# jens-nau/NeRF-VO

Hardware: AMD Instinct MI355X
Metric: training ray-samples/sec (higher is better)
Workload: dtype f16; 1 GPU; BASELINE configs[1]: Replica-shaped full mapping step, depth-nerfacto (proposal sampling 256/96/48), fixed poses; normal_supervision=False, loss_scale=GradScaler 65536 dynamic, skipped_zero_weight_heads=True, rays_per_gpu=4096, samples_per_ray=48, keyframes=192, sampler=proposal-network (nerfacto), parallelism=single GPU (no process group)

## Files before the change

include/nerfvo_hip.h:

```cpp
#ifndef NERFVO_HIP_H
#define NERFVO_HIP_H

#include <stddef.h>
#include <stdint.h>

#ifdef __cplusplus
extern "C" {
#endif

#define NVO_OK 0
#define NVO_ERR_INVALID 1
#define NVO_ERR_HIP 2
#define NVO_ERR_UNSUPPORTED 3

typedef struct nvo_module_s* nvo_module_t;
typedef void* nvo_stream_t;

const char* nvo_last_error(void);
int nvo_version(void);
int nvo_profile_enable(int on);
int64_t nvo_profile_summary(char* buf, uint64_t buf_size);

int nvo_create_encoding(uint32_t n_input_dims, const char* encoding_json, nvo_module_t* out);
int nvo_create_network(uint32_t n_input_dims, uint32_t n_output_dims, const char* network_json,
// ... 132 lines not shown
    uint32_t R, S, S_out;
    const void* pre;
    uint32_t pre_stride;
    const float* x01;
    const float* sbins;
    const float* tbins;
    float density_bias;
    float* sigma;
    float* weights;
    float anneal, histogram_padding, near_plane, far_plane;
    const float* jitter;
    float* sbins_out;
    float* tbins_out;
    const float* anneal_dev;
    const float* origins;
    const float* directions;
    float* x01_out;
    int act_bf16;
} nvo_weights_pdf_args;
int nvo_weights_pdf(nvo_stream_t stream, const nvo_weights_pdf_args* args);

typedef struct nvo_main_loss_args {
    uint32_t R, S;
    const void* pre;
    uint32_t pre_stride;
    const void* rgb;
    uint32_t rgb_stride;
    const float* x01;
    const float* sbins;
    const float* tbins;
    float density_bias;
    const float* gt_rgb;
    const float* gt_depth;
    const float* directions_norm;
    float rgb_mult, distortion_mult, depth_mult, depth_sigma;
    float inv_rays;
    float depth_level_div;
    float loss_scale;
    float* out_rgb;
    float* out_depth;
    float* out_expected_depth;
    float* out_accumulation;
    float* weights;
    float* losses;
    void* dpre;
    uint32_t dpre_stride;
    void* drgb;
    uint32_t drgb_stride;
    const float* dsigma_dx;
    float dsigma_inv_scale;
    const float* gt_normal;
    float normal_mult;
    float* out_normals;
    int act_bf16;
    const float* loss_scale_dev;
    uint32_t* nonfinite_flag;
    uint8_t* tile_live;
} nvo_main_loss_args;
int nvo_main_render_loss(nvo_stream_t stream, const nvo_main_loss_args* args);

typedef struct nvo_prop_loss_args {
    uint32_t R, S, S_main;
    const void* pre;
    uint32_t pre_stride;
    const float* x01;
    const float* sbins;
    const float* tbins;
    const float* sbins_main;
    const float* weights_main;
    float density_bias;
    const float* gt_depth;
    const float* directions_norm;
    float interlevel_mult, depth_mult, depth_sigma;
    float inv_rays, depth_level_div, loss_scale;
    float* losses;
    void* dpre;
    uint32_t dpre_stride;
    int act_bf16;
    const float* loss_scale_dev;
    uint32_t* nonfinite_flag;
} nvo_prop_loss_args;
int nvo_prop_loss(nvo_stream_t stream, const nvo_prop_loss_args* args);
int nvo_prop_loss_pair(nvo_stream_t stream, const nvo_prop_loss_args* args0, const nvo_prop_loss_args* args1);

typedef struct nvo_color_args {
    uint32_t R, S;
    const void* sh;
    const void* base_out;
    const void* embedding;
    const int32_t* cam_idx;
    const void* weights;
    void* rgb;
    void* hidden;
    const void* drgb;
    void* d_base_out;
    float* d_embedding;
    float* d_sh;
    float* d_weights;
    int act_bf16;
    void* det_scratch;
    uint64_t det_scratch_bytes;
    uint32_t n_cameras;
    uint32_t* nonfinite_flag;
    float* dw_replicas;
    uint32_t n_dw_replicas;
    const uint8_t* tile_live;
    const float* tile_live_count;
} nvo_color_args;
int nvo_nerfacto_color_fwd(nvo_stream_t stream, const nvo_color_args* args);
int nvo_nerfacto_color_bwd(nvo_stream_t stream, const nvo_color_args* args);
uint64_t nvo_color_det_scratch_bytes(uint32_t R, uint32_t S);

uint64_t nvo_occ_march_scratch_bytes(uint32_t R);
int nvo_occ_march(nvo_stream_t stream, uint32_t R, const float* origins, const float* directions,
                  const uint8_t* bitfield, int n_levels, float cone_angle, float t_near, const float* jitter,
                  uint32_t capacity, uint32_t* counts, uint32_t* offsets, int32_t* ray_idx, float* t_out,
                  float* dt_out, void* scratch, uint64_t scratch_bytes);
int nvo_occ_march_resume(nvo_stream_t stream, uint32_t R, const float* origins, const float* directions,
                         const uint8_t* bitfield, int n_levels, float cone_angle, float t_near, const float* jitter,
                         uint32_t capacity, uint32_t* counts, uint32_t* offsets, int32_t* ray_idx, float* t_out,
                         float* dt_out, void* scratch, uint64_t scratch_bytes, const float* t_resume, uint32_t max_new,
                         float* t_next);
int nvo_occ_march_runs(nvo_stream_t stream, uint32_t R, const float* origins, const float* directions,
                       const uint8_t* bitfield, int n_levels, float cone_angle, float t_near, const float* jitter,
                       uint32_t* counts, void* scratch, uint64_t scratch_bytes, const float* t_resume, uint32_t max_new,
                       float* t_next, const uint32_t* R_dev, uint32_t run_offset);
int nvo_occ_pack(nvo_stream_t stream, uint32_t R, const uint32_t* counts_in, uint32_t capacity, uint32_t* counts_out,
                 uint32_t* offsets, uint32_t* totals, const void* scratch, uint64_t scratch_bytes, int32_t* ray_idx,
                 float* t_out, float* dt_out, const uint32_t* R_dev, uint32_t run_offset);
uint64_t nvo_occ_pack_state_bytes(void);
int nvo_occ_pack_fused(nvo_stream_t stream, uint32_t R, const uint32_t* counts_in, uint32_t capacity, uint32_t* counts_out,
                       uint32_t* offsets, uint32_t* totals, const void* scratch, uint64_t scratch_bytes, int32_t* ray_idx,
                       float* t_out, float* dt_out, const uint32_t* R_dev, uint32_t run_offset, void* state,
                       const float* origins, const float* directions, float aabb_lo, float aabb_hi, float* x01,
                       uint32_t rays_per_group );
int nvo_occ_update(nvo_stream_t stream, int n_levels, float* grid, const float* fresh, float decay,
                   float threshold, uint8_t* bitfield, void* scratch8);
int nvo_occ_cell_positions(nvo_stream_t stream, int level, const float* jitter, float* positions);
int nvo_occ_mark_untrained(nvo_stream_t stream, int n_levels, float* grid, uint32_t n_images, const float* intrinsics,
                           const float* c2w, uint32_t H, uint32_t W, float margin);
int nvo_occ_sample_cells(nvo_stream_t stream, uint32_t n, uint32_t first, uint32_t n_total, uint32_t step, uint32_t seed,
                         uint32_t stream_id, int n_levels, const float* grid, float thresh, float aabb_lo, float aabb_hi,
                         float* x01, uint32_t* cell_idx);

typedef struct nvo_ngp_rgb_args {
    uint32_t capacity;
    const void* sh;
    const void* density_out;
    const int32_t* ray_idx;
    const void* weights;
    void* rgb_out;
    void* hidden;
    const void* d_rgb_out;
    void* d_density_out;
    const float* d_density_pre;
    float* d_weights;
    uint32_t* nonfinite_flag;
    float* dw_replicas;
    uint32_t n_dw_replicas;
} nvo_ngp_rgb_args;
int nvo_ngp_rgb_fwd(nvo_stream_t stream, const nvo_ngp_rgb_args* args);
int nvo_ngp_rgb_bwd(nvo_stream_t stream, const nvo_ngp_rgb_args* args);

typedef struct nvo_ngp_loss_args {
    uint32_t R, capacity;
    const uint32_t* counts;
// ... 209 lines not shown
```

nerf-vo_amd/_lib.py:

```python
from __future__ import annotations

import ctypes as C
import os
from pathlib import Path

PKG_DIR = Path(__file__).resolve().parent
LIB_PATH = PKG_DIR / "lib" / "libnerfvo_hip.so"

_lib = None

_u32, _u64, _i64, _int = C.c_uint32, C.c_uint64, C.c_int64, C.c_int
_i32 = C.c_int32
_p = C.c_void_p
_f = C.c_float


class WeightsPdfArgs(C.Structure):
    _fields_ = [("R", _u32), ("S", _u32), ("S_out", _u32), ("pre", _p), ("pre_stride", _u32), ("x01", _p),
                ("sbins", _p), ("tbins", _p), ("density_bias", _f), ("sigma", _p), ("weights", _p),
                ("anneal", _f), ("histogram_padding", _f), ("near_plane", _f), ("far_plane", _f),
                ("jitter", _p), ("sbins_out", _p), ("tbins_out", _p), ("anneal_dev", _p),
                ("origins", _p), ("directions", _p), ("x01_out", _p), ("act_bf16", _int)]


# ... 69 lines not shown
                ("nonfinite_flag", _p), ("dw_replicas", _p), ("n_dw_replicas", _u32)]


class NgpLossArgs(C.Structure):
    _fields_ = [("R", _u32), ("capacity", _u32), ("counts", _p), ("offsets", _p), ("ray_idx", _p), ("t", _p), ("dt", _p),
                ("density_out", _p), ("density_stride", _u32), ("rgb_out", _p), ("rgb_stride", _u32),
                ("background", _p), ("gt_rgb", _p), ("gt_depth", _p), ("directions_norm", _p), ("rgb_mult", _f),
                ("depth_mult", _f), ("inv_rays", _f), ("loss_scale", _f), ("out_rgb", _p), ("out_depth", _p),
                ("out_accumulation", _p), ("losses", _p), ("d_rgb_out", _p), ("d_rgb_stride", _u32),
                ("d_density_pre", _p), ("carry_in", _p), ("carry_out", _p), ("accumulate_outputs", _u32),
                ("train_min_transmittance", _f), ("gt_depth_cov", _p), ("ray_state", _p), ("R_dev", _p), ("world_size", _u32)]


class NgpAliveArgs(C.Structure):
    _fields_ = [("R", _u32), ("counts", _p), ("offsets", _p), ("dt", _p), ("density_out", _p), ("density_stride", _u32),
                ("min_transmittance", _f), ("kept", _p), ("state", _p), ("R_dev", _p), ("resume_in", _p), ("carry_in", _p),
                ("kept_base", _u32), ("t_next", _p), ("resume_out", _p), ("carry_out", _p)]


class TsdfArgs(C.Structure):
    _fields_ = [("tsdf", _p), ("weight", _p), ("color", _p), ("frames", _p), ("depth", _p), ("rgb", _p),
                ("nx", _u32), ("ny", _u32), ("nz", _u32), ("K", _u32), ("H", _u32), ("W", _u32),
                ("lower_x", _f), ("lower_y", _f), ("lower_z", _f), ("voxel_size", _f), ("trunc", _f), ("depth_max", _f)]


TSDF_MAX_FRAMES = 16


class NnArgs(C.Structure):
    _fields_ = [("points", _p), ("point_index", _p), ("cell_start", _p), ("queries", _p), ("out_dist2", _p), ("out_index", _p),
                ("N", _u32), ("M", _u32), ("gx", _u32), ("gy", _u32), ("gz", _u32),
                ("lower_x", _f), ("lower_y", _f), ("lower_z", _f), ("cell_size", _f), ("max_dist", _f),
                ("has_xf", _i32), ("xf", _f * 12)]


NN_MAX_CELLS_PER_AXIS = 1024


_SIGNATURES = {
    "nvo_last_error": (C.c_char_p, []),
    "nvo_version": (_int, []),
    "nvo_profile_enable": (_int, [_int]),
    "nvo_profile_summary": (_i64, [C.c_char_p, _u64]),
    "nvo_create_encoding": (_int, [_u32, C.c_char_p, C.POINTER(_p)]),
    "nvo_create_network": (_int, [_u32, _u32, C.c_char_p, C.POINTER(_p)]),
    "nvo_create_network_with_input_encoding": (_int, [_u32, _u32, C.c_char_p, C.c_char_p, C.POINTER(_p)]),
    "nvo_destroy": (_int, [_p]),
    "nvo_n_input_dims": (_u32, [_p]),
    "nvo_n_output_dims": (_u32, [_p]),
    "nvo_padded_output_dims": (_u32, [_p]),
    "nvo_n_params": (_u64, [_p]),
    "nvo_initial_params": (_int, [_p, _u64, _p]),
    "nvo_ctx_bytes": (_u64, [_p, _u32]),
    "nvo_set_option": (_int, [_p, C.c_char_p, _i64]),
    "nvo_fwd": (_int, [_p, _p, _u32, _p, _p, _p, _p]),
    "nvo_bwd": (_int, [_p, _p, _u32, _p, _p, _p, _p, _p, _p, _p]),
    "nvo_bwd_fork": (_int, [_p, _p, _p, _u32, _p, _p, _p, _p, _p, _p, _p]),
    "nvo_grid_describe": (_int, [_p, _p, _p]),
    "nvo_grid_indices": (_int, [_p, _p, _u32, _p, _p]),
    "nvo_raygen": (_int, [_p, _u32, _p, _p, _p, _p, _p, _p, _p, _p, _p]),
    "nvo_se3_exp_map": (_int, [_p, _u32, _p, _p]),
    "nvo_pose_exp_map": (_int, [_p, _u32, _p, _p, _int]),
    "nvo_positions_bwd": (_int, [_p, _u32, _u32, _p, _p, _p, _p, _p, _p]),
    "nvo_sh_bwd_input_f32": (_int, [_p, _u32, _u32, _p, _p, _p]),
    "nvo_pose_bwd": (_int, [_p, _u32, _p, _p, _p, _p, _p, _p, _p]),
    "nvo_se3_exp_map_bwd": (_int, [_p, _u32, _p, _p, _f, _f, _f, _p, _p, _int]),
    "nvo_se3_exp_map_bwd_scaled": (_int, [_p, _u32, _p, _p, _f, _f, _f, _p, _p, _int, _p]),
    "nvo_gather_pixels": (_int, [_p, _u32, _p, _u32, _u32, _u32, _p, _p]),
    "nvo_sample_lindisp": (_int, [_p, _u32, _u32, _f, _f, _p, _p, _p]),
    "nvo_sample_pixels": (_int, [_p, _u32, _u32, _p, _p, _p, _p, _u32]),
    "nvo_lindisp_positions": (_int, [_p, _u32, _u32, _f, _f, _p, _p, _p, _p, _p, _p]),
    "nvo_gather_targets": (_int, [_p, _u32, _p, _u32, _u32, _p, _p, _p, _p, _p, _p, _p, _p]),
    "nvo_sample_positions": (_int, [_p, _u32, _u32, _p, _p, _p, _p]),
    "nvo_dirs01": (_int, [_p, _u32, _p, _p]),
    "nvo_sh_encode": (_int, [_p, _u32, _u32, _p, _p]),
    "nvo_sh_encode_t": (_int, [_p, _u32, _u32, _p, _p, _int]),
    "nvo_ray_head": (_int, [_p, C.POINTER(RayHeadArgs)]),
    "nvo_rays_given": (_int, [_p, _u32, _p, _p, _p, _p, _u32, _u32, _p, _p, _p, _p, _p, _p, _p, _p, _p, _p, _p, _p, _p, _p]),
    "nvo_ray_head_zero": (_int, [_p, C.POINTER(RayHeadArgs), _u32, _p, _p]),
    "nvo_weights_pdf": (_int, [_p, C.POINTER(WeightsPdfArgs)]),
    "nvo_main_render_loss": (_int, [_p, C.POINTER(MainLossArgs)]),
    "nvo_prop_loss": (_int, [_p, C.POINTER(PropLossArgs)]),
    "nvo_prop_loss_pair": (_int, [_p, _p, _p]),
    "nvo_nerfacto_color_fwd": (_int, [_p, C.POINTER(ColorArgs)]),
    "nvo_nerfacto_color_bwd": (_int, [_p, C.POINTER(ColorArgs)]),
    "nvo_color_det_scratch_bytes": (_u64, [_u32, _u32]),
    "nvo_pose_bwd_cams": (_int, [_p, _u32, _p, _p, _p, _p, _p, _p, _p, _u32]),
    "nvo_pose_bwd_det": (_int, [_p, _u32, _p, _p, _p, _p, _p, _p, _p, _p, _u32]),
    "nvo_occ_march_scratch_bytes": (_u64, [_u32]),
    "nvo_occ_march": (_int, [_p, _u32, _p, _p, _p, _int, _f, _f, _p, _u32, _p, _p, _p, _p, _p, _p, _u64]),
    "nvo_occ_march_resume": (_int, [_p, _u32, _p, _p, _p, _int, _f, _f, _p, _u32, _p, _p, _p, _p, _p, _p, _u64, _p, _u32, _p]),
    "nvo_occ_update": (_int, [_p, _int, _p, _p, _f, _f, _p, _p]),
    "nvo_occ_cell_positions": (_int, [_p, _int, _p, _p]),
    "nvo_occ_mark_untrained": (_int, [_p, _int, _p, _u32, _p, _p, _u32, _u32, _f]),
    "nvo_occ_sample_cells": (_int, [_p, _u32, _u32, _u32, _u32, _u32, _u32, _int, _p, _f, _f, _f, _p, _p]),
    "nvo_occ_march_runs": (_int, [_p, _u32, _p, _p, _p, _int, _f, _f, _p, _p, _p, _u64, _p, _u32, _p, _p, _u32]),
    "nvo_occ_pack": (_int, [_p, _u32, _p, _u32, _p, _p, _p, _p, _u64, _p, _p, _p, _p, _u32]),
    "nvo_occ_pack_state_bytes": (_u64, []),
    "nvo_occ_pack_fused": (_int, [_p, _u32, _p, _u32, _p, _p, _p, _p, _u64, _p, _p, _p, _p, _u32, _p, _p, _p, _f, _f, _p, _u32]),
    "nvo_ngp_count_alive": (_int, [_p, C.POINTER(NgpAliveArgs)]),
    "nvo_ngp_positions_live": (_int, [_p, _u32, _p, _p, _p, _p, _f, _f, _p, _p]),
    "nvo_ngp_positions_bwd_dev": (_int, [_p, _u32, _u32, _p, _p, _p, _p, _p, _f, _f, _p, _p, _p, _p]),
    "nvo_ngp_positions": (_int, [_p, _u32, _p, _p, _p, _p, _f, _f, _p]),
    "nvo_depth_align_scratch_bytes": (_u64, [_u32, _u32]),
    "nvo_depth_align": (_int, [_p, C.POINTER(DepthAlignArgs)]),
    "nvo_ngp_positions_bwd": (_int, [_p, _u32, _u32, _p, _p, _p, _p, _p, _f, _f, _p, _p, _p]),
    "nvo_ngp_rgb_fwd": (_int, [_p, C.POINTER(NgpRgbArgs)]),
    "nvo_ngp_rgb_bwd": (_int, [_p, C.POINTER(NgpRgbArgs)]),
    "nvo_ngp_composite_loss": (_int, [_p, C.POINTER(NgpLossArgs)]),
    "nvo_ngp_thickness": (_int, [_p, _u32, _p, _u32, _int, _p]),
    "nvo_ngp_thickness_splat": (_int, [_p, _u32, _p, _u32, _p, _p]),
    "nvo_fill_i32": (_int, [_p, _u32, _p, _i32]),
    "nvo_tsdf_integrate": (_int, [_p, C.POINTER(TsdfArgs)]),
    "nvo_nn_query": (_int, [_p, C.POINTER(NnArgs)]),
    "nvo_adam_step": (_int, [_p, _u64, _p, _p, _p, _int, _p, _p, _f, _f, _f, _f, _u32, _f, _f, _p, _p]),
    "nvo_write_floats": (_int, [_p, _p, _u32, _p]),
    "nvo_nonfinite_flag": (_int, [_p, _u64, _p, _int, _p]),
    "nvo_nonfinite_flag_or": (_int, [_p, _u64, _p, _int, _p]),
    "nvo_adam_step_groups": (_int, [_p, _u32, _p, _p, _p, _p, _int, _p, _p, _f, _f, _f, _f, _f, _p]),
    "nvo_nonfinite_flag_ranges": (_int, [_p, _u32, _p, _p, _p, _int, _p]),
    "nvo_nonfinite_flag_ranges_or": (_int, [_p, _u32, _p, _p, _p, _int, _p]),
    "nvo_nonfinite_flag_spans_or": (_int, [_p, _u32, _p, _p, _p, _p, _int, _p]),
    "nvo_cast_half": (_int, [_p, _u64, _p, _p]),
    "nvo_zero_ranges": (_int, [_p, _u32, _p, _p]),
    "nvo_bwd_zero_ranges": (_int, [_p, _p, _p, _p, _u32]),
    "nvo_fold_replicas": (_int, [_p, _u32, _p, _p, _p, _p]),
    "nvo_fused_adam_range": (_int, [_p, _p, _p]),
    "nvo_set_fused_adam": (_int, [_p, _p]),
    "nvo_ema_update": (_int, [_p, _u64, _p, _p, _p, _f, _u32, _p]),
    "nvo_ema_update_dev": (_int, [_p, _u64, _p, _p, _p, _f, _p, _p]),
    "nvo_ema_update_dev_part": (_int, [_p, _u64, _p, _p, _p, _f, _p, _p]),
    "nvo_cast_working_copy": (_int, [_p, _u64, _p, _p, _u32, _p, _p]),
    "nvo_adam_step_groups_mixed": (_int, [_p, _u32, _p, _p, _p, _p, _int, _p, _p, _f, _f, _f, _f, _f, _p, _u32, _p, _p]),
    "nvo_adam_step_groups_scaled": (_int, [_p, _u32, _p, _p, _p, _p, _int, _p, _p, _f, _f, _f, _f, _f, _p, _u32, _p, _p, _p]),
    "nvo_adam_step_groups_tail": (_int, [_p, _u32, _p, _p, _p, _p, _int, _p, _p, _f, _f, _f, _f, _f, _p, _u32, _p, _p, _p, _p]),
    "nvo_opt_commit_write": (_int, [_p, _u32, _u32, _u32, _p, _p, _p, _p, _f, _f, _u32, _f, _f, _p, _f, _f, _p, _u32, _p]),
    "nvo_opt_commit_table": (_int, [_p, _u32, _u32, _u32, _p, _p, _p, _p, _f, _f, _u32, _f, _f, _p, _f, _f, _p, _p, _u32, _p]),
    "nvo_opt_commit": (_int, [_p, _u32, _u32, _u32, _p, _p, _p, _p, _f, _f, _u32, _f, _f, _p, _f, _f]),
    "nvo_cast_bf16": (_int, [_p, _u64, _p, _p]),
    "nvo_cast_shards": (_int, [_p, _u64, _u32, _u32, _p, _p, _int, _p]),
    "nvo_flag_from_wire": (_int, [_p, _p, _p]),
}


def exported_symbols() -> list[str]:
    return sorted(_SIGNATURES)


def lib() -> C.CDLL:
    global _lib
    if _lib is None:
        if not LIB_PATH.exists():
            raise RuntimeError(
                f"{LIB_PATH} is missing: the HIP extension has not been built. "
                "Run `python -c 'import __graft_entry__ as g; g.build()'` (or `python nerf-vo_amd/build.py`). "
                "There is no CPU fallback."
            )
        import torch

        handle = C.CDLL(str(LIB_PATH), mode=getattr(os, "RTLD_NOW", 2))
        for name, (restype, argtypes) in _SIGNATURES.items():
            fn = getattr(handle, name)
            fn.restype = restype
            fn.argtypes = argtypes
        _lib = handle
    return _lib
# ... 7 lines not shown
```

nerf-vo_amd/csrc/render.hip:

```cpp
#include "nvo_kernels.h"
#include "../../include/nerfvo_hip.h"

#include <float.h>

namespace {

constexpr int kRayBlock = 256;
constexpr int kRaysPerBlock = kRayBlock / 64;
constexpr int kMaxS = 256;
constexpr float kLossEps = 1.0e-7f;

__device__ __forceinline__ float wave_incl_scan(float v, int) { return nvo_wave_incl_scan(v); }
__device__ __forceinline__ float wave_sum(float v) { return nvo_wave_sum(v); }

__device__ __forceinline__ float nan_to_num(float v) {
    if (isnan(v)) return 0.f;
    if (isinf(v)) return v > 0.f ? FLT_MAX : -FLT_MAX;
    return v;
}

__device__ __forceinline__ float spacing_fn(float x) { return x < 1.f ? x * 0.5f : 1.f - 1.f / (2.f * x); }
__device__ __forceinline__ float spacing_fn_inv(float x) { return x < 0.5f ? 2.f * x : 1.f / (2.f - 2.f * x); }

__device__ __forceinline__ int upper_bound(const float* a, int n, float v) {
// ... 409 lines not shown
    const float* x01 = a.x01 + 3 * so;
    ray_weights(lane, S, pre, bf, a.pre_stride, x01, tb, a.density_bias, nullptr, w, Tr);
    __builtin_amdgcn_fence(__ATOMIC_RELEASE, "wavefront");
    __builtin_amdgcn_wave_barrier();
    __builtin_amdgcn_fence(__ATOMIC_ACQUIRE, "wavefront");

    float carry = 0.f;
    for (uint32_t base = 0; base < S; base += 64) {
        const uint32_t i = base + lane;
        const float v = (i < S) ? w[i] : 0.f;
        const float incl = wave_incl_scan(v, lane) + carry;
        if (i < S) cy[i + 1] = incl;
        carry = nvo_wave_bcast(incl, 63);
    }
    if (lane == 0) cy[0] = 0.f;
    for (uint32_t i = lane; i < S + 2; i += 64) g[i] = 0.f;
    __builtin_amdgcn_fence(__ATOMIC_RELEASE, "wavefront");
    __builtin_amdgcn_wave_barrier();
    __builtin_amdgcn_fence(__ATOMIC_ACQUIRE, "wavefront");

    float l_inter = 0.f;
    if ((uint32_t)lane < Sm) {
        const float* cm = a.sbins_main + (size_t)r * (Sm + 1);
        const float wm = a.weights_main[(size_t)r * Sm + lane];
        int lo = upper_bound(sb, (int)S, cm[lane]) - 1;
        lo = min(max(lo, 0), (int)S - 1);
        int hi = upper_bound(sb + 1, (int)S, cm[lane + 1]);
        hi = min(max(hi, 0), (int)S - 1);
        const float w_outer = cy[hi + 1] - cy[lo];
        const float diff = wm - w_outer;
        if (diff > 0.f) {
            l_inter = diff * diff / (wm + kLossEps);
            const float coef = a.interlevel_mult * a.inv_rays / (float)Sm;
            const float gi = -2.f * diff / (wm + kLossEps) * coef;
            atomicAdd(&g[lo], gi);
            atomicAdd(&g[hi + 1], -gi);
        }
    }
    l_inter = wave_sum(l_inter) * a.inv_rays / (float)Sm;
    __builtin_amdgcn_fence(__ATOMIC_RELEASE, "wavefront");
    __builtin_amdgcn_wave_barrier();
    __builtin_amdgcn_fence(__ATOMIC_ACQUIRE, "wavefront");
    float l_depth = 0.f;
    const bool use_depth = a.depth_mult != 0.f && a.gt_depth;
    const float z = use_depth ? a.gt_depth[r] * a.directions_norm[r] : 0.f;
    const float mask = z > 0.f ? 1.f : 0.f;
    carry = 0.f;
    for (uint32_t base = 0; base < S; base += 64) {
        const uint32_t i = base + lane;
        const float v = (i < S) ? g[i] : 0.f;
        const float incl = wave_incl_scan(v, lane) + carry;
        carry = nvo_wave_bcast(incl, 63);
        float gi = incl;
        if (i < S && use_depth) {
            const float midp = 0.5f * (tb[i] + tb[i + 1]);
            const float len = tb[i + 1] - tb[i];
            const float gss = __expf(-((midp - z) * (midp - z)) / (2.f * a.depth_sigma)) * len * mask;
            l_depth += -__logf(w[i] + kLossEps) * gss;
            gi += a.depth_mult * a.depth_level_div * a.inv_rays * (-gss / (w[i] + kLossEps));
        }
        if (i < S) g[i] = gi;
    }
    l_depth = wave_sum(l_depth) * a.inv_rays * a.depth_level_div;
    if (lane == 0) {
        float* shard = a.losses + 8 * (r & 63u);
        atomicAdd(shard + 0, a.interlevel_mult * l_inter);
        atomicAdd(shard + 1, a.depth_mult * l_depth);
    }
    if (a.dpre == nullptr) return;
    __builtin_amdgcn_fence(__ATOMIC_RELEASE, "wavefront");
    __builtin_amdgcn_wave_barrier();
    __builtin_amdgcn_fence(__ATOMIC_ACQUIRE, "wavefront");
    const bool overflow = ray_weights_bwd(lane, S, pre, bf, a.pre_stride, x01, tb, a.density_bias, w, Tr, g, a.loss_scale,
                                          (nvo_h16*)a.dpre + so * a.dpre_stride, a.dpre_stride, true);
    if (a.nonfinite_flag && __ballot(overflow) != 0ull && lane == 0) atomicOr(a.nonfinite_flag, 1u);
    if (a.dpre_stride != 16) {
        for (uint32_t i = lane; i < S; i += 64) {
            nvo_h16* dp = (nvo_h16*)a.dpre + (so + i) * a.dpre_stride;
            for (uint32_t k = 1; k < a.dpre_stride; ++k) dp[k] = (nvo_h16)0;
        }
    }
}

}

extern "C" {

int nvo_weights_pdf(nvo_stream_t stream, const nvo_weights_pdf_args* args) {
    NVO_REQUIRE(args != nullptr, "weights_pdf: args is NULL");
    const nvo_weights_pdf_args a = *args;
    NVO_REQUIRE(a.S >= 1 && a.S <= (uint32_t)kMaxS, "weights_pdf: samples per ray %u not in 1..%d", a.S, kMaxS);
    NVO_REQUIRE(a.S_out <= (uint32_t)kMaxS, "weights_pdf: S_out %u > %d", a.S_out, kMaxS);
    NVO_REQUIRE(a.S_out == 0 || (a.sbins_out && a.tbins_out), "weights_pdf: output bins are NULL");
    NVO_REQUIRE(a.pre && a.x01 && a.tbins && a.weights && a.sbins, "weights_pdf: NULL input");
    NVO_REQUIRE(!a.x01_out || (a.origins && a.directions && a.S_out > 0), "weights_pdf: x01_out needs origins, directions and S_out");
    if (a.R == 0) return NVO_OK;
    NVO_PROF(stream, "weights_pdf[S%u]", a.S);
    NVO_LAUNCH(k_weights_pdf, dim3(nvo_div_up(a.R, kRaysPerBlock)), dim3(kRayBlock), 0,
                       (hipStream_t)stream, a);
    NVO_CHECK_LAUNCH();
    return NVO_OK;
}

int nvo_main_render_loss(nvo_stream_t stream, const nvo_main_loss_args* args) {
    NVO_REQUIRE(args != nullptr, "main_render_loss: args is NULL");
    const nvo_main_loss_args a = *args;
    NVO_REQUIRE(a.S >= 1 && a.S <= 64, "main_render_loss: samples per ray %u not in 1..64", a.S);
    NVO_REQUIRE(a.pre && a.rgb && a.x01 && a.sbins && a.tbins && a.out_rgb && a.out_depth &&
                a.out_accumulation, "main_render_loss: NULL input/output");
    NVO_REQUIRE(!a.dpre || (a.drgb && a.losses && a.gt_rgb && a.drgb_stride >= 3),
                "main_render_loss: training mode needs drgb, losses, gt_rgb");
    NVO_REQUIRE(!a.tile_live || (a.dpre && (a.S & 15u) == 0u), "main_render_loss: tile_live needs training mode and S %% 16 == 0 (S = %u)", a.S);
    if (a.R == 0) return NVO_OK;
    NVO_PROF(stream, "main_render_loss");
    NVO_LAUNCH(k_main_render_loss, dim3(nvo_div_up(a.R, kRaysPerBlock)), dim3(kRayBlock), 0,
                       (hipStream_t)stream, a);
    NVO_CHECK_LAUNCH();
    return NVO_OK;
}

int nvo_prop_loss(nvo_stream_t stream, const nvo_prop_loss_args* args) {
    NVO_REQUIRE(args != nullptr, "prop_loss: args is NULL");
    const nvo_prop_loss_args a = *args;
    NVO_REQUIRE(a.S >= 1 && a.S <= (uint32_t)kMaxS && a.S_main >= 1 && a.S_main <= 64,
                "prop_loss: S=%u (<=%d) S_main=%u (<=64)", a.S, kMaxS, a.S_main);
    NVO_REQUIRE(a.pre && a.x01 && a.sbins && a.tbins && a.sbins_main && a.weights_main && a.losses &&
                (a.dpre == nullptr || a.dpre_stride >= 1), "prop_loss: NULL input/output");
    if (a.R == 0) return NVO_OK;
    NVO_PROF(stream, "prop_loss[S%u]", a.S);
    const uint32_t blocks = nvo_div_up(a.R, kRaysPerBlock);
    NVO_LAUNCH(k_prop_loss, dim3(blocks), dim3(kRayBlock), 0, (hipStream_t)stream, a, a, blocks);
    NVO_CHECK_LAUNCH();
    return NVO_OK;
}

int nvo_prop_loss_pair(nvo_stream_t stream, const nvo_prop_loss_args* args0, const nvo_prop_loss_args* args1) {
    NVO_REQUIRE(args0 != nullptr && args1 != nullptr, "prop_loss_pair: args is NULL");
    for (const nvo_prop_loss_args* p : {args0, args1}) {
        const nvo_prop_loss_args& a = *p;
        NVO_REQUIRE(a.S >= 1 && a.S <= (uint32_t)kMaxS && a.S_main >= 1 && a.S_main <= 64,
                    "prop_loss_pair: S=%u (<=%d) S_main=%u (<=64)", a.S, kMaxS, a.S_main);
        NVO_REQUIRE(a.pre && a.x01 && a.sbins && a.tbins && a.sbins_main && a.weights_main && a.losses &&
                    (a.dpre == nullptr || a.dpre_stride >= 1), "prop_loss_pair: NULL input/output");
    }
    const uint32_t b0 = nvo_div_up(args0->R, kRaysPerBlock), b1 = nvo_div_up(args1->R, kRaysPerBlock);
    if (b0 + b1 == 0) return NVO_OK;
    NVO_PROF(stream, "prop_loss[S%u+S%u]", args0->S, args1->S);
    NVO_LAUNCH(k_prop_loss, dim3(b0 + b1), dim3(kRayBlock), 0, (hipStream_t)stream, *args0, *args1, b0);
    NVO_CHECK_LAUNCH();
    return NVO_OK;
}

}
```

Before: 385.5 million ray-samples/s.

## Add register-prefetched variants of per-ray weight, render-loss and proposal-loss kernels

Adds v1 versions of the weights_pdf, main_render_loss and prop_loss kernels. Each one issues all per-ray global loads (pre-activations, x01, bins, colors, ground truth) up front into registers, using clamped or safe-pointer loads so no loads depend on branches, then computes weights and gradients from those registers. The goal is to hide global-memory latency behind the scan work in these wave-per-ray kernels. The v1 kernels are the default, and a runtime switch can select the old ones. Holding all chunks for up to 256 samples in registers raises register pressure, which may cut occupancy.

```diff
diff --git a/include/nerfvo_hip.h b/include/nerfvo_hip.h
--- a/include/nerfvo_hip.h
+++ b/include/nerfvo_hip.h
@@ -238,6 +238,7 @@
 } nvo_prop_loss_args;
 int nvo_prop_loss(nvo_stream_t stream, const nvo_prop_loss_args* args);
 int nvo_prop_loss_pair(nvo_stream_t stream, const nvo_prop_loss_args* args0, const nvo_prop_loss_args* args1);
+int nvo_set_ray_kernel_form(int form);
 
 typedef struct nvo_color_args {
     uint32_t R, S;
diff --git a/nerf-vo_amd/_lib.py b/nerf-vo_amd/_lib.py
--- a/nerf-vo_amd/_lib.py
+++ b/nerf-vo_amd/_lib.py
@@ -175,6 +175,7 @@
     "nvo_main_render_loss": (_int, [_p, C.POINTER(MainLossArgs)]),
     "nvo_prop_loss": (_int, [_p, C.POINTER(PropLossArgs)]),
     "nvo_prop_loss_pair": (_int, [_p, _p, _p]),
+    "nvo_set_ray_kernel_form": (_int, [_int]),
     "nvo_nerfacto_color_fwd": (_int, [_p, C.POINTER(ColorArgs)]),
     "nvo_nerfacto_color_bwd": (_int, [_p, C.POINTER(ColorArgs)]),
     "nvo_color_det_scratch_bytes": (_u64, [_u32, _u32]),
diff --git a/nerf-vo_amd/csrc/render.hip b/nerf-vo_amd/csrc/render.hip
--- a/nerf-vo_amd/csrc/render.hip
+++ b/nerf-vo_amd/csrc/render.hip
@@ -515,9 +515,574 @@
     }
 }
 
+constexpr int kMaxChunks = kMaxS / 64;
+
+__device__ __forceinline__ float cvt_raw16(nvo_h16 raw, bool bf) {
+    return bf ? __uint_as_float((uint32_t)raw << 16) : (float)__builtin_bit_cast(_Float16, raw);
+}
+
+template <int NC>
+struct RayIn {
+    float x0[NC], t0[NC], t1[NC];
+    nvo_h16 pr[NC];
+};
+
+template <int NC>
+__device__ __forceinline__ void ray_load(RayIn<NC>& in, int lane, uint32_t S, const nvo_h16* pre, uint32_t pre_stride,
+                                         const float* x01, const float* tb) {
+#pragma unroll
+    for (int c = 0; c < NC; ++c) {
+        const uint32_t i = min(64u * c + (uint32_t)lane, S - 1u);
+        in.x0[c] = x01[3 * (size_t)i];
+        in.pr[c] = pre[(size_t)i * pre_stride];
+        in.t0[c] = tb[i];
+        in.t1[c] = tb[i + 1];
+    }
+}
+
+__device__ __forceinline__ float ld_or(bool use, const float* p, const float* safe) { return *(use ? p : safe); }
+
+__device__ __forceinline__ void bins_row_load(float (&v)[kMaxChunks + 1], int lane, uint32_t S, const float* row) {
+#pragma unroll
+    for (int c = 0; c <= kMaxChunks; ++c) {
+        v[c] = row[min(64u * c + (uint32_t)lane, S)];
+    }
+}
+__device__ __forceinline__ void bins_row_stage(const float (&v)[kMaxChunks + 1], int lane, uint32_t S, float* dst) {
+#pragma unroll
+    for (int c = 0; c <= kMaxChunks; ++c) {
+        const uint32_t i = 64u * c + (uint32_t)lane;
+        if (i <= S) dst[i] = v[c];
+    }
+}
+
+template <int NC>
+__device__ __forceinline__ void ray_weights_regs(int lane, uint32_t S, const RayIn<NC>& in, bool bf, float bias,
+                                                 float* __restrict__ sigma_out, float* w, float* Tr) {
+    float carry = 0.f;
+#pragma unroll
+    for (int c = 0; c < NC; ++c) {
+        const uint32_t base = 64u * c;
+        if (base >= S) break;
+        const uint32_t i = base + lane;
+        float dd = 0.f, sg = 0.f;
+        if (i < S) {
+            const bool sel = in.x0[c] > 0.f;
+            sg = sel ? __expf(fminf(cvt_raw16(in.pr[c], bf) + bias, 60.f)) : 0.f;
+            dd = (in.t1[c] - in.t0[c]) * sg;
+            if (sigma_out) sigma_out[i] = sg;
+        }
+        const float incl = wave_incl_scan(dd, lane) + carry;
+        const float T = __expf(-(incl - dd));
+        if (i < S) {
+            w[i] = nan_to_num((1.f - __expf(-dd)) * T);
+            Tr[i] = T;
+        }
+        carry = nvo_wave_bcast(incl, 63);
+    }
+}
+
+template <int NC>
+__device__ __forceinline__ bool ray_weights_bwd_regs(int lane, uint32_t S, const RayIn<NC>& in, bool bf, float bias,
+                                                     const float* w, const float* Tr, const float* g,
+                                                     float loss_scale, nvo_h16* __restrict__ dpre,
+                                                     uint32_t dpre_stride, bool zero_row = false,
+                                                     unsigned long long* live = nullptr) {
+    bool overflow = false;
+    const float fmt_max = bf ? 3.0e38f : 65504.0f;
+    float total = 0.f;
+    for (uint32_t base = 0; base < S; base += 64) {
+        const uint32_t i = base + lane;
+        total += (i < S) ? g[i] * w[i] : 0.f;
+    }
+    total = wave_sum(total);
+    float carry = 0.f;
+#pragma unroll
+    for (int c = 0; c < NC; ++c) {
+        const uint32_t base = 64u * c;
+        if (base >= S) break;
+        const uint32_t i = base + lane;
+        const float gw = (i < S) ? g[i] * w[i] : 0.f;
+        const float incl = wave_incl_scan(gw, lane) + carry;
+        if (i < S) {
+            const bool sel = in.x0[c] > 0.f;
+            float d = 0.f;
+            if (sel) {
+                const float x = cvt_raw16(in.pr[c], bf) + bias;
+                const float delta = in.t1[c] - in.t0[c];
+                const float dsig = delta * (g[i] * (Tr[i] - w[i]) - (total - incl));
+                d = dsig * __expf(fminf(fmaxf(x, -15.f), 15.f));
+            }
+            overflow = overflow || !(fabsf(d * loss_scale) <= fmt_max);
+            const nvo_h16 d16 = nvo_cvt16(d * loss_scale, bf);
+            if (live) *live = __ballot((d16 & 0x7fffu) != 0u);
+            if (zero_row && dpre_stride == 16) {
+                uint4 lo = make_uint4(0u, 0u, 0u, 0u);
+                lo.x = (uint32_t)d16;
+                uint4* row = reinterpret_cast<uint4*>(dpre + (size_t)i * 16);
+                row[0] = lo;
+                row[1] = make_uint4(0u, 0u, 0u, 0u);
+            } else {
+                dpre[(size_t)i * dpre_stride] = d16;
+            }
+        }
+        carry = nvo_wave_bcast(incl, 63);
+    }
+    return overflow;
+}
+
+__global__ void __launch_bounds__(kRayBlock)
+k_weights_pdf_v1(nvo_weights_pdf_args a) {
+    __shared__ float lds[kRaysPerBlock][4][kMaxS + 4];
+    const int lane = threadIdx.x & 63, wib = threadIdx.x >> 6;
+    const uint32_t r = blockIdx.x * kRaysPerBlock + wib;
+    if (r >= a.R) return;
+    float* w = lds[wib][0];
+    float* Tr = lds[wib][1];
+    float* cdf = lds[wib][2];
+    float* sb = lds[wib][3];
+    const uint32_t S = a.S;
+    const size_t so = (size_t)r * S;
+    const bool bf = a.act_bf16 != 0;
+    const bool resample = a.S_out != 0;
+
+    const float* tb = a.tbins + (size_t)r * (S + 1);
+    RayIn<kMaxChunks> in;
+    ray_load(in, lane, S, (const nvo_h16*)a.pre + so * a.pre_stride, a.pre_stride, a.x01 + 3 * so, tb);
+    float sbv[kMaxChunks + 1];
+    bins_row_load(sbv, lane, S, resample ? a.sbins + (size_t)r * (S + 1) : tb);
+    const float jit = ld_or(resample && a.jitter, a.jitter + r, tb);
+    const bool positions = resample && a.x01_out;
+    float o[3], d[3];
+#pragma unroll
+    for (int k = 0; k < 3; ++k) {
+        o[k] = ld_or(positions, a.origins + 3 * (size_t)r + k, tb);
+        d[k] = ld_or(positions, a.directions + 3 * (size_t)r + k, tb);
+    }
+    float anneal = a.anneal;
+    if (resample && a.anneal_dev) anneal = *a.anneal_dev;
+
+    ray_weights_regs(lane, S, in, bf, a.density_bias, a.sigma ? a.sigma + so : nullptr, w, Tr);
+    for (uint32_t i = lane; i < S; i += 64) a.weights[so + i] = w[i];
+    if (!resample) return;
+
+    float part = 0.f;
+    for (uint32_t i = lane; i < S; i += 64) {
+        const float wa = (anneal == 1.0f ? w[i] : powf(w[i], anneal)) + a.histogram_padding;
+        Tr[i] = wa;
+        part += wa;
+    }
+    float sum = wave_sum(part);
+    const float padding = fmaxf(1e-5f - sum, 0.f);
+    sum += padding;
+    const float pad_each = padding / (float)S;
+    float carry = 0.f;
+    for (uint32_t base = 0; base < S; base += 64) {
+        const uint32_t i = base + lane;
+        const float p = (i < S) ? (Tr[i] + pad_each) / sum : 0.f;
+        const float incl = wave_incl_scan(p, lane) + carry;
+        if (i < S) cdf[i + 1] = fminf(1.f, incl);
+        carry = nvo_wave_bcast(incl, 63);
+    }
+    if (lane == 0) cdf[0] = 0.f;
+    bins_row_stage(sbv, lane, S, sb);
+    __builtin_amdgcn_fence(__ATOMIC_RELEASE, "wavefront");
+    __builtin_amdgcn_wave_barrier();
+    __builtin_amdgcn_fence(__ATOMIC_ACQUIRE, "wavefront");
+
+    const uint32_t nb = a.S_out + 1;
+    const float inv_nb = 1.0f / (float)nb;
+    const float shift = a.jitter ? jit * inv_nb : 0.5f * inv_nb;
+    const float s_near = spacing_fn(a.near_plane), s_far = spacing_fn(a.far_plane);
+    for (uint32_t j = lane; j < nb; j += 64) {
+        const float u = (float)j * inv_nb + shift;
+        const int inds = upper_bound(cdf, (int)S + 1, u);
+        const int below = min(max(inds - 1, 0), (int)S), above = min(max(inds, 0), (int)S);
+        const float c0 = cdf[below], c1 = cdf[above];
+        float t = (u - c0) / (c1 - c0);
+        if (isnan(t)) t = 0.f;
+        t = fminf(fmaxf(t, 0.f), 1.f);
+        const float b = sb[below] + t * (sb[above] - sb[below]);
+        const float tv = spacing_fn_inv(b * s_far + (1.f - b) * s_near);
+        a.sbins_out[(size_t)r * nb + j] = b;
+        a.tbins_out[(size_t)r * nb + j] = tv;
+        if (a.x01_out) w[j] = tv;
+    }
+    if (a.x01_out) {
+        __builtin_amdgcn_fence(__ATOMIC_RELEASE, "wavefront");
+        __builtin_amdgcn_wave_barrier();
+        __builtin_amdgcn_fence(__ATOMIC_ACQUIRE, "wavefront");
+        for (uint32_t j = lane; j < a.S_out; j += 64) {
+            float p[3];
+            nvo_contract_position01(o, d, (w[j] + w[j + 1]) * 0.5f, p);
+            float* xo = a.x01_out + 3 * ((size_t)r * a.S_out + j);
+            xo[0] = p[0]; xo[1] = p[1]; xo[2] = p[2];
+        }
+    }
+}
+
+__global__ void __launch_bounds__(kRayBlock)
+k_main_render_loss_v1(nvo_main_loss_args a) {
+    __shared__ float lds[kRaysPerBlock][4][64 + 4];
+    const int lane = threadIdx.x & 63, wib = threadIdx.x >> 6;
+    const uint32_t r = blockIdx.x * kRaysPerBlock + wib;
+    if (r >= a.R) return;
+    if (a.loss_scale_dev) a.loss_scale = *a.loss_scale_dev;
+    float* w = lds[wib][0];
+    float* Tr = lds[wib][1];
+    float* g = lds[wib][2];
+    float* ut = lds[wib][3];
+    const uint32_t S = a.S;
+    const size_t so = (size_t)r * S;
+    const bool bf = a.act_bf16 != 0;
+    const bool act = (uint32_t)lane < S;
+    const bool train = a.dpre != nullptr;
+    const bool has_normals = a.dsigma_dx != nullptr;
+    const bool use_dist = train && a.distortion_mult != 0.f;
+    const bool use_depth = train && a.depth_mult != 0.f && a.gt_depth;
+    const bool use_gt_normal = train && has_normals && a.gt_normal && a.normal_mult != 0.f;
+
+    const float* tb = a.tbins + (size_t)r * (S + 1);
+    RayIn<1> in;
+    ray_load(in, lane, S, (const nvo_h16*)a.pre + so * a.pre_stride, a.pre_stride, a.x01 + 3 * so, tb);
+    const uint32_t ic = min((uint32_t)lane, S - 1u);
+    nvo_h16 craw[3];
+    {
+        const nvo_h16* cp = (const nvo_h16*)a.rgb + (so + ic) * a.rgb_stride;
+        craw[0] = cp[0]; craw[1] = cp[1]; craw[2] = cp[2];
+    }
+    const float* sb = a.sbins + (size_t)r * (S + 1);
+    const float s0 = ld_or(use_dist, sb + ic, tb), s1 = ld_or(use_dist, sb + ic + 1, tb);
+    float gp[3], gt[3], q[3];
+#pragma unroll
+    for (int k = 0; k < 3; ++k) {
+        gp[k] = ld_or(has_normals, a.dsigma_dx + 3 * (so + ic) + k, tb);
+        gt[k] = ld_or(train, a.gt_rgb + 3 * (size_t)r + k, tb);
+        q[k] = ld_or(use_gt_normal, a.gt_normal + 3 * (size_t)r + k, tb);
+    }
+    const float zg = ld_or(use_depth, a.gt_depth + r, tb), dn = ld_or(use_depth, a.directions_norm + r, tb);
+
+    ray_weights_regs(lane, S, in, bf, a.density_bias, nullptr, w, Tr);
+    const float wi = act ? w[lane] : 0.f;
+    if (a.weights && act) a.weights[so + lane] = wi;
+
+    float c[3] = {0.f, 0.f, 0.f};
+    if (act) {
+        c[0] = cvt_raw16(craw[0], bf); c[1] = cvt_raw16(craw[1], bf); c[2] = cvt_raw16(craw[2], bf);
+    }
+    const float acc = wave_sum(wi);
+    float pix[3], clast[3];
+#pragma unroll
+    for (int k = 0; k < 3; ++k) {
+        clast[k] = nvo_wave_bcast(c[k], (int)S - 1);
+        pix[k] = wave_sum(wi * c[k]) + clast[k] * (1.f - acc);
+    }
+    const float mid = act ? 0.5f * (in.t0[0] + in.t1[0]) : 0.f;
+    const float cum = wave_incl_scan(wi, lane);
+    const unsigned long long ballot = __ballot(act && cum >= 0.5f);
+    const int med = ballot ? (int)__builtin_ctzll(ballot) : (int)S - 1;
+    const float depth_med = nvo_wave_bcast(mid, med);
+    if (lane == 0) {
+        a.out_rgb[3 * (size_t)r + 0] = pix[0];
+        a.out_rgb[3 * (size_t)r + 1] = pix[1];
+        a.out_rgb[3 * (size_t)r + 2] = pix[2];
+        a.out_depth[r] = depth_med;
+        a.out_accumulation[r] = acc;
+    }
+    if (a.out_expected_depth) {
+        const float num = wave_sum(wi * mid);
+        if (lane == 0) a.out_expected_depth[r] = num / (acc + 1e-10f);
+    }
+    float nrm[3] = {0.f, 0.f, 0.f};
+    float Nv[3] = {0.f, 0.f, 0.f}, Nhat[3] = {0.f, 0.f, 0.f};
+    float rN = 0.f;
+    if (has_normals) {
+        if (act) {
+            const float gx = gp[0] * a.dsigma_inv_scale, gy = gp[1] * a.dsigma_inv_scale,
+                        gz = gp[2] * a.dsigma_inv_scale;
+            const float inv = -1.f / fmaxf(sqrtf(gx * gx + gy * gy + gz * gz), 1e-12f);
+            nrm[0] = gx * inv; nrm[1] = gy * inv; nrm[2] = gz * inv;
+        }
+#pragma unroll
+        for (int k = 0; k < 3; ++k) Nv[k] = wave_sum(wi * nrm[k]);
+        rN = sqrtf(Nv[0] * Nv[0] + Nv[1] * Nv[1] + Nv[2] * Nv[2]);
+#pragma unroll
+        for (int k = 0; k < 3; ++k) Nhat[k] = Nv[k] / (rN + 1e-10f);
+        if (a.out_normals && lane == 0) {
+#pragma unroll
+            for (int k = 0; k < 3; ++k) a.out_normals[3 * (size_t)r + k] = 0.5f * (Nhat[k] + 1.f);
+        }
+    }
+    if (!train) return;
+
+    float dpix[3];
+    float l_rgb = 0.f;
+#pragma unroll
+    for (int k = 0; k < 3; ++k) {
+        const float e = pix[k] - gt[k];
+        l_rgb += e * e;
+        dpix[k] = a.rgb_mult * 2.f * e * a.inv_rays * (1.f / 3.f);
+    }
+    l_rgb *= a.inv_rays * (1.f / 3.f);
+    float gw = 0.f;
+    float dc[3] = {0.f, 0.f, 0.f};
+    if (act) {
+#pragma unroll
+        for (int k = 0; k < 3; ++k) {
+            gw += dpix[k] * (c[k] - clast[k]);
+            dc[k] = dpix[k] * wi;
+        }
+        if ((uint32_t)lane == S - 1) {
+#pragma unroll
+            for (int k = 0; k < 3; ++k) dc[k] += dpix[k] * (1.f - acc);
+        }
+    }
+    float l_dist = 0.f;
+    if (use_dist) {
+        const float uti = act ? 0.5f * (s0 + s1) : 0.f;
+        if (act) ut[lane] = uti;
+        __builtin_amdgcn_fence(__ATOMIC_RELEASE, "wavefront");
+        __builtin_amdgcn_wave_barrier();
+        __builtin_amdgcn_fence(__ATOMIC_ACQUIRE, "wavefront");
+        float inner = 0.f;
+        if (act) {
+            for (uint32_t j = 0; j < S; ++j) inner += w[j] * fabsf(uti - ut[j]);
+        }
+        const float ds = act ? (s1 - s0) : 0.f;
+        l_dist = wave_sum(wi * inner + wi * wi * ds * (1.f / 3.f)) * a.inv_rays;
+        if (act) gw += a.distortion_mult * a.inv_rays * (2.f * inner + 2.f * wi * ds * (1.f / 3.f));
+    }
+    float l_depth = 0.f;
+    if (use_depth) {
+        const float z = zg * dn;
+        const float mask = z > 0.f ? 1.f : 0.f;
+        float term = 0.f;
+        if (act) {
+            const float len = in.t1[0] - in.t0[0];
+            const float gss = __expf(-((mid - z) * (mid - z)) / (2.f * a.depth_sigma)) * len * mask;
+            term = -__logf(wi + kLossEps) * gss;
+            gw += a.depth_mult * a.depth_level_div * a.inv_rays * (-gss / (wi + kLossEps));
+        }
+        l_depth = wave_sum(term) * a.inv_rays * a.depth_level_div;
+    }
+    float l_normal = 0.f;
+    if (use_gt_normal) {
+        float sh[3], p[3], dp[3];
+        float rs = 0.f, rq = 0.f;
+#pragma unroll
+        for (int k = 0; k < 3; ++k) {
+            sh[k] = 0.5f * (Nhat[k] + 1.f);
+            rs += sh[k] * sh[k];
+            rq += q[k] * q[k];
+        }
+        rs = fmaxf(sqrtf(rs), 1e-12f);
+        rq = fmaxf(sqrtf(rq), 1e-12f);
+        float pdq = 0.f;
+#pragma unroll
+        for (int k = 0; k < 3; ++k) {
+            p[k] = sh[k] / rs;
+            q[k] /= rq;
+            l_normal += fabsf(p[k] - q[k]);
+            pdq += p[k] * q[k];
+        }
+        l_normal = (l_normal + 1.f - pdq) * a.inv_rays;
+        float pdp = 0.f;
+#pragma unroll
+        for (int k = 0; k < 3; ++k) {
+            const float e = p[k] - q[k];
+            dp[k] = a.normal_mult * a.inv_rays * ((e > 0.f ? 1.f : (e < 0.f ? -1.f : 0.f)) - q[k]);
+            pdp += p[k] * dp[k];
+        }
+        float dN[3], NdN = 0.f;
+#pragma unroll
+        for (int k = 0; k < 3; ++k) {
+            dN[k] = 0.5f * (dp[k] - p[k] * pdp) / rs;
+            NdN += Nv[k] * dN[k];
+        }
+        const float den = rN + 1e-10f;
+        const float radial = rN > 0.f ? NdN / (rN * den * den) : 0.f;
+        if (act) {
+#pragma unroll
+            for (int k = 0; k < 3; ++k) gw += (dN[k] / den - Nv[k] * radial) * nrm[k];
+        }
+    }
+    if (lane == 0) {
+        float* shard = a.losses + 8 * (r & 63u);
+        atomicAdd(shard + 0, a.rgb_mult * l_rgb);
+        atomicAdd(shard + 1, a.distortion_mult * l_dist);
+        atomicAdd(shard + 2, a.depth_mult * l_depth);
+        if (l_normal != 0.f) atomicAdd(shard + 6, a.normal_mult * l_normal);
+    }
+    if (act) g[lane] = gw;
+    __builtin_amdgcn_fence(__ATOMIC_RELEASE, "wavefront");
+    __builtin_amdgcn_wave_barrier();
+    __builtin_amdgcn_fence(__ATOMIC_ACQUIRE, "wavefront");
+    unsigned long long pre_live = 0ull;
+    bool overflow = ray_weights_bwd_regs(lane, S, in, bf, a.density_bias, w, Tr, g, a.loss_scale,
+                                         (nvo_h16*)a.dpre + so * a.dpre_stride, a.dpre_stride, false, &pre_live);
+    if (act) {
+        const float fmt_max = bf ? 3.0e38f : 65504.0f;
+#pragma unroll
+        for (int k = 0; k < 3; ++k) overflow = overflow || !(fabsf(dc[k] * a.loss_scale) <= fmt_max);
+    }
+    if (a.nonfinite_flag && __ballot(overflow) != 0ull && lane == 0) atomicOr(a.nonfinite_flag, 1u);
+    bool rgb_nz = false;
+    if (act && a.drgb_stride == 16) {
+        uint4 lo = make_uint4(0u, 0u, 0u, 0u);
+        lo.x = nvo_cvt16x2(dc[0] * a.loss_scale, dc[1] * a.loss_scale, bf);
+        lo.y = (uint32_t)nvo_cvt16(dc[2] * a.loss_scale, bf);
+        uint4* row = reinterpret_cast<uint4*>((nvo_h16*)a.drgb + (so + lane) * 16);
+        row[0] = lo;
+        row[1] = make_uint4(0u, 0u, 0u, 0u);
+        rgb_nz = ((lo.x | lo.y) & 0x7fff7fffu) != 0u;
+    } else if (act) {
+        nvo_h16* dp = (nvo_h16*)a.drgb + (so + lane) * a.drgb_stride;
+#pragma unroll
+        for (int k = 0; k < 3; ++k) {
+            dp[k] = nvo_cvt16(dc[k] * a.loss_scale, bf);
+            rgb_nz = rgb_nz || (dp[k] & 0x7fffu) != 0u;
+        }
+        for (uint32_t k = 3; k < a.drgb_stride; ++k) dp[k] = (nvo_h16)0;
+    }
+    if (a.tile_live) {
+        const unsigned long long rgb_live = __ballot(rgb_nz);
+        uint32_t byte = 0u;
+        if (lane < (int)(S >> 4)) {
+            const uint32_t sh = 16u * (uint32_t)lane;
+            byte = (((rgb_live >> sh) & 0xffffull) != 0ull ? 1u : 0u) | (((pre_live >> sh) & 0xffffull) != 0ull ? 2u : 0u);
+            a.tile_live[(so >> 4) + lane] = (uint8_t)byte;
+        }
+        const uint32_t n_live_tiles = (uint32_t)__popcll(__ballot(byte != 0u));
+        if (lane == 0 && n_live_tiles) atomicAdd(a.losses + 8 * (r & 63u) + 7, (float)n_live_tiles);
+    }
+}
+
+__global__ void __launch_bounds__(kRayBlock)
+k_prop_loss_v1(nvo_prop_loss_args a0, nvo_prop_loss_args a1, uint32_t blocks0) {
+    __shared__ float lds[kRaysPerBlock][5][kMaxS + 4];
+    const int lane = threadIdx.x & 63, wib = threadIdx.x >> 6;
+    const bool second = blockIdx.x >= blocks0;
+    nvo_prop_loss_args a = second ? a1 : a0;
+    const uint32_t r = (second ? blockIdx.x - blocks0 : blockIdx.x) * kRaysPerBlock + wib;
+    if (r >= a.R) return;
+    if (a.loss_scale_dev) a.loss_scale = *a.loss_scale_dev;
+    float* w = lds[wib][0];
+    float* Tr = lds[wib][1];
+    float* g = lds[wib][2];
+    float* cy = lds[wib][3];
+    float* sb = lds[wib][4];
+    const uint32_t S = a.S, Sm = a.S_main;
+    const size_t so = (size_t)r * S;
+    const bool bf = a.act_bf16 != 0;
+    const bool use_depth = a.depth_mult != 0.f && a.gt_depth;
+
+    const float* tb = a.tbins + (size_t)r * (S + 1);
+    RayIn<kMaxChunks> in;
+    ray_load(in, lane, S, (const nvo_h16*)a.pre + so * a.pre_stride, a.pre_stride, a.x01 + 3 * so, tb);
+    float sbv[kMaxChunks + 1];
+    bins_row_load(sbv, lane, S, a.sbins + (size_t)r * (S + 1));
+    const uint32_t lm = min((uint32_t)lane, Sm - 1u);
+    const float cm0 = a.sbins_main[(size_t)r * (Sm + 1) + lm];
+    const float cm1 = a.sbins_main[(size_t)r * (Sm + 1) + lm + 1];
+    const float wm = a.weights_main[(size_t)r * Sm + lm];
+    const float zg = ld_or(use_depth, a.gt_depth + r, tb), dn = ld_or(use_depth, a.directions_norm + r, tb);
+
+    ray_weights_regs(lane, S, in, bf, a.density_bias, nullptr, w, Tr);
+    bins_row_stage(sbv, lane, S, sb);
+    __builtin_amdgcn_fence(__ATOMIC_RELEASE, "wavefront");
+    __builtin_amdgcn_wave_barrier();
+    __builtin_amdgcn_fence(__ATOMIC_ACQUIRE, "wavefront");
+
+    float carry = 0.f;
+    for (uint32_t base = 0; base < S; base += 64) {
+        const uint32_t i = base + lane;
+        const float v = (i < S) ? w[i] : 0.f;
+        const float incl = wave_incl_scan(v, lane) + carry;
+        if (i < S) cy[i + 1] = incl;
+        carry = nvo_wave_bcast(incl, 63);
+    }
+    if (lane == 0) cy[0] = 0.f;
+    for (uint32_t i = lane; i < S + 2; i += 64) g[i] = 0.f;
+    __builtin_amdgcn_fence(__ATOMIC_RELEASE, "wavefront");
+    __builtin_amdgcn_wave_barrier();
+    __builtin_amdgcn_fence(__ATOMIC_ACQUIRE, "wavefront");
+
+    float l_inter = 0.f;
+    if ((uint32_t)lane < Sm) {
+        int lo = upper_bound(sb, (int)S, cm0) - 1;
+        lo = min(max(lo, 0), (int)S - 1);
+        int hi = upper_bound(sb + 1, (int)S, cm1);
+        hi = min(max(hi, 0), (int)S - 1);
+        const float w_outer = cy[hi + 1] - cy[lo];
+        const float diff = wm - w_outer;
+        if (diff > 0.f) {
+            l_inter = diff * diff / (wm + kLossEps);
+            const float coef = a.interlevel_mult * a.inv_rays / (float)Sm;
+            const float gi = -2.f * diff / (wm + kLossEps) * coef;
+            atomicAdd(&g[lo], gi);
+            atomicAdd(&g[hi + 1], -gi);
+        }
+    }
+    l_inter = wave_sum(l_inter) * a.inv_rays / (float)Sm;
+    __builtin_amdgcn_fence(__ATOMIC_RELEASE, "wavefront");
+    __builtin_amdgcn_wave_barrier();
+    __builtin_amdgcn_fence(__ATOMIC_ACQUIRE, "wavefront");
+    float l_depth = 0.f;
+    const float z = use_depth ? zg * dn : 0.f;
+    const float mask = z > 0.f ? 1.f : 0.f;
+    carry = 0.f;
+#pragma unroll
+    for (int c = 0; c < kMaxChunks; ++c) {
+        const uint32_t base = 64u * c;
+        if (base >= S) break;
+        const uint32_t i = base + lane;
+        const float v = (i < S) ? g[i] : 0.f;
+        const float incl = wave_incl_scan(v, lane) + carry;
+        carry = nvo_wave_bcast(incl, 63);
+        float gi = incl;
+        if (i < S && use_depth) {
+            const float midp = 0.5f * (in.t0[c] + in.t1[c]);
+            const float len = in.t1[c] - in.t0[c];
+            const float gss = __expf(-((midp - z) * (midp - z)) / (2.f * a.depth_sigma)) * len * mask;
+            l_depth += -__logf(w[i] + kLossEps) * gss;
+            gi += a.depth_mult * a.depth_level_div * a.inv_rays * (-gss / (w[i] + kLossEps));
+        }
+        if (i < S) g[i] = gi;
+    }
+    l_depth = wave_sum(l_depth) * a.inv_rays * a.depth_level_div;
+    if (lane == 0) {
+        float* shard = a.losses + 8 * (r & 63u);
+        atomicAdd(shard + 0, a.interlevel_mult * l_inter);
+        atomicAdd(shard + 1, a.depth_mult * l_depth);
+    }
+    if (a.dpre == nullptr) return;
+    __builtin_amdgcn_fence(__ATOMIC_RELEASE, "wavefront");
+    __builtin_amdgcn_wave_barrier();
+    __builtin_amdgcn_fence(__ATOMIC_ACQUIRE, "wavefront");
+    const bool overflow = ray_weights_bwd_regs(lane, S, in, bf, a.density_bias, w, Tr, g, a.loss_scale,
+                                               (nvo_h16*)a.dpre + so * a.dpre_stride, a.dpre_stride, true);
+    if (a.nonfinite_flag && __ballot(overflow) != 0ull && lane == 0) atomicOr(a.nonfinite_flag, 1u);
+    if (a.dpre_stride != 16) {
+        for (uint32_t i = lane; i < S; i += 64) {
+            nvo_h16* dp = (nvo_h16*)a.dpre + (so + i) * a.dpre_stride;
+            for (uint32_t k = 1; k < a.dpre_stride; ++k) dp[k] = (nvo_h16)0;
+        }
+    }
+}
+
+int g_ray_form = -1;
+constexpr bool kWeightsPdfForm1 = true, kMainLossForm1 = true, kPropLossForm1 = true;
+inline bool use_form1(bool kernel_default) { return g_ray_form < 0 ? kernel_default : g_ray_form != 0; }
+
 }
 
 extern "C" {
+
+int nvo_set_ray_kernel_form(int form) {
+    NVO_REQUIRE(form >= -1 && form <= 1, "set_ray_kernel_form: form %d not 0, 1 or -1 (every kernel's default)", form);
+    g_ray_form = form;
+    return NVO_OK;
+}
 
 int nvo_weights_pdf(nvo_stream_t stream, const nvo_weights_pdf_args* args) {
     NVO_REQUIRE(args != nullptr, "weights_pdf: args is NULL");
@@ -529,8 +1094,10 @@
     NVO_REQUIRE(!a.x01_out || (a.origins && a.directions && a.S_out > 0), "weights_pdf: x01_out needs origins, directions and S_out");
     if (a.R == 0) return NVO_OK;
     NVO_PROF(stream, "weights_pdf[S%u]", a.S);
-    NVO_LAUNCH(k_weights_pdf, dim3(nvo_div_up(a.R, kRaysPerBlock)), dim3(kRayBlock), 0,
-                       (hipStream_t)stream, a);
+    if (use_form1(kWeightsPdfForm1))
+        NVO_LAUNCH(k_weights_pdf_v1, dim3(nvo_div_up(a.R, kRaysPerBlock)), dim3(kRayBlock), 0, (hipStream_t)stream, a);
+    else
+        NVO_LAUNCH(k_weights_pdf, dim3(nvo_div_up(a.R, kRaysPerBlock)), dim3(kRayBlock), 0, (hipStream_t)stream, a);
     NVO_CHECK_LAUNCH();
     return NVO_OK;
 }
@@ -546,8 +1113,10 @@
     NVO_REQUIRE(!a.tile_live || (a.dpre && (a.S & 15u) == 0u), "main_render_loss: tile_live needs training mode and S %% 16 == 0 (S = %u)", a.S);
     if (a.R == 0) return NVO_OK;
     NVO_PROF(stream, "main_render_loss");
-    NVO_LAUNCH(k_main_render_loss, dim3(nvo_div_up(a.R, kRaysPerBlock)), dim3(kRayBlock), 0,
-                       (hipStream_t)stream, a);
+    if (use_form1(kMainLossForm1))
+        NVO_LAUNCH(k_main_render_loss_v1, dim3(nvo_div_up(a.R, kRaysPerBlock)), dim3(kRayBlock), 0, (hipStream_t)stream, a);
+    else
+        NVO_LAUNCH(k_main_render_loss, dim3(nvo_div_up(a.R, kRaysPerBlock)), dim3(kRayBlock), 0, (hipStream_t)stream, a);
     NVO_CHECK_LAUNCH();
     return NVO_OK;
 }
@@ -562,7 +1131,10 @@
     if (a.R == 0) return NVO_OK;
     NVO_PROF(stream, "prop_loss[S%u]", a.S);
     const uint32_t blocks = nvo_div_up(a.R, kRaysPerBlock);
-    NVO_LAUNCH(k_prop_loss, dim3(blocks), dim3(kRayBlock), 0, (hipStream_t)stream, a, a, blocks);
+    if (use_form1(kPropLossForm1))
+        NVO_LAUNCH(k_prop_loss_v1, dim3(blocks), dim3(kRayBlock), 0, (hipStream_t)stream, a, a, blocks);
+    else
+        NVO_LAUNCH(k_prop_loss, dim3(blocks), dim3(kRayBlock), 0, (hipStream_t)stream, a, a, blocks);
     NVO_CHECK_LAUNCH();
     return NVO_OK;
 }
@@ -579,7 +1151,10 @@
     const uint32_t b0 = nvo_div_up(args0->R, kRaysPerBlock), b1 = nvo_div_up(args1->R, kRaysPerBlock);
     if (b0 + b1 == 0) return NVO_OK;
     NVO_PROF(stream, "prop_loss[S%u+S%u]", args0->S, args1->S);
-    NVO_LAUNCH(k_prop_loss, dim3(b0 + b1), dim3(kRayBlock), 0, (hipStream_t)stream, *args0, *args1, b0);
+    if (use_form1(kPropLossForm1))
+        NVO_LAUNCH(k_prop_loss_v1, dim3(b0 + b1), dim3(kRayBlock), 0, (hipStream_t)stream, *args0, *args1, b0);
+    else
+        NVO_LAUNCH(k_prop_loss, dim3(b0 + b1), dim3(kRayBlock), 0, (hipStream_t)stream, *args0, *args1, b0);
     NVO_CHECK_LAUNCH();
     return NVO_OK;
 }
```

New measurement: 389.2 million ray-samples/s, median of 6. About the same (+1.0%).
